# nkargas/Gen2-UHF-RFID-Reader

Measured on AMD Instinct MI355X. Metric: I/Q Msamples/s through matched_filter->gate->tag_decoder (+ EPC decodes/s), 40 kHz FM0, higher is better.
Workload: dtype f32; 1 GPU; configs[1]: batch of 1024 noise-replicas per GPU of the 71-round file_source_test stand-in trace, FM0 40 kHz BLF @ 2 Msps (1076066 raw I/Q samples each, sigma=0.002), generated and resident in HBM; streams_per_gpu=1024, hbm_bytes_traces=8815132672, parallelism=traces sharded per GPU, no collective

## Files before the change

gen2-uhf-rfid-reader_amd/csrc/rfid_capi.hip:

```cpp
#include <hip/hip_runtime.h>

#include <cmath>
#include <ctime>
#include <pthread.h>
#include <cstdio>
#include <cstdlib>
#include <cstring>
#include <deque>
#include <initializer_list>
#include <map>
#include <memory>
#include <new>
#include <vector>

#include "rfid_host_math.h"
#include "rfid_kernels.hpp"
#include "rfid_inventory.hpp"
#include "rfid_tracks.hpp"
#include "rfid_quality.hpp"
#include "rfid_mi355x.h"
#include "rfid_gen2_host.h"
#define LS2_LAUNCH(kernel, gx, gy, block, args) \
  hipLaunchKernelGGL(rfidk::kernel, dim3((unsigned)(gx), (unsigned)(gy)), dim3((unsigned)(block)), 0, ls2_stream, args)
static thread_local hipStream_t ls2_stream = nullptr;
static thread_local unsigned ls2_front_lds = 0;
#define LS2_LAUNCH_FRONT(kernel, gx, gy, block, args) \
  hipLaunchKernelGGL(rfidk::kernel, dim3((unsigned)(gx), (unsigned)(gy)), dim3((unsigned)(block)), ls2_front_lds, ls2_stream, args)
static double g_la_t[20] = {0};
static long g_la_n[20] = {0};
static bool g_la_on = false;
static inline void la_count(int k, double dt) { if (g_la_on) { g_la_t[k] += dt; g_la_n[k]++; } }
static inline double la_now() { struct timespec ts; clock_gettime(CLOCK_MONOTONIC, &ts); return 1e3 * (double)ts.tv_sec + 1e-6 * (double)ts.tv_nsec; }
struct LaTimer { int k; double t0; explicit LaTimer(int kk) : k(kk), t0(g_la_on ? la_now() : 0.0) {} ~LaTimer() { if (g_la_on) la_count(k, la_now() - t0); } };
#include "rfid_ls2_enqueue.hpp"

using namespace rfidk;

namespace {

struct DevBuf {
  void *p = nullptr;
  size_t cap = 0;
};

}

struct RfidKnobs {
  int long_stream = 1;
  int overlap = 1;
  int ls_calibrate = 1;
  int ls_debug = 0;
  int la_profile = 0;
  int front_unfused = 0;
  int front_chunks = 1;
  int fsm_lanes_min = -1;
  int dc_rounds = -1;
  int la_upload_kernel = 1;
  int front_lds_kb = -1;
  int inventory_slots = 0;
};

struct rfid_ctx {
  rfid_params prm;
  RfidKnobs knobs;
  int device = 0;
  hipStream_t stream = nullptr;
  char err[512];
  float t_cand[N_TCAND];

  rfid_reader_state rs;

  void *d_small = nullptr;
  GateState *d_gate1 = nullptr;
  int *d_io = nullptr;
  DevBuf s_in, s_out;
  DevBuf synth_tab;
  DevBuf ls2_ws;
  DevBuf ls2_ws_alt;
  bool ls2_mark_failed = false;
  bool y_touched = false;
  Ls2Ctl *ls2_host = nullptr;
  Ls2Ctl *d_ls2_ctl = nullptr;
  int ls2_P = 0;
  int ls2_rounds[3] = {0, 0, 0};
  bool ls2_generous = false;
  int ls_mode = 1;
// ... 184 lines not shown
  float front_ms = 0.0f;
};

namespace {

void sio_free(rfid_ctx *c);
int sio_process(rfid_ctx *c, int b, int64_t n_new, bool flush);
int sio_submit(rfid_ctx *c, int b, int64_t n_new, bool flush);
int sio_collect(rfid_ctx *c);
void la_free(rfid_ctx *c);
int la_mf_work(rfid_ctx *c, const rfid_cf32 *in, int n_in, rfid_cf32 *out, int out_cap, int *n_produced);
int la_gate_work(rfid_ctx *c, const rfid_cf32 *in, int n_in, rfid_cf32 *out, int out_cap, int *n_consumed, int *n_written);
int la_gate_swallow(rfid_ctx *c, const rfid_cf32 *in, int n_in, rfid_cf32 *out, int out_cap, int *n_consumed, int *n_written);
bool la_decoder_result(rfid_ctx *c, const rfid_cf32 *in, int wlen, int type, rfid_decode_result *r);

int fail(rfid_ctx *c, int code, const char *what, hipError_t e = hipSuccess) {
  if (c) {
    if (e != hipSuccess)
      snprintf(c->err, sizeof(c->err), "%s: %s", what, hipGetErrorString(e));
    else
      snprintf(c->err, sizeof(c->err), "%s", what);
  }
  return code;
}

struct KnobEntry { const char *name, *env; int RfidKnobs::*field; int lo, hi; };
const KnobEntry g_knob_table[] = {
  {"long_stream", "RFID_LONG_STREAM", &RfidKnobs::long_stream, 0, 2},
  {"overlap", "RFID_OVERLAP", &RfidKnobs::overlap, 0, 2},
  {"ls_calibrate", "RFID_LS_CALIBRATE", &RfidKnobs::ls_calibrate, 0, 1},
  {"ls_debug", "RFID_LS_DEBUG", &RfidKnobs::ls_debug, 0, 1},
  {"la_profile", "RFID_LA_PROFILE", &RfidKnobs::la_profile, 0, 1},
  {"front_unfused", "RFID_FRONT_UNFUSED", &RfidKnobs::front_unfused, 0, 1},
  {"front_chunks", "RFID_FRONT_CHUNKS", &RfidKnobs::front_chunks, 1, rfid_ctx::MAX_CHUNKS},
  {"fsm_lanes_min", "RFID_LS2_FSM_LANES_MIN", &RfidKnobs::fsm_lanes_min, -1, 1 << 30},
  {"dc_rounds", "RFID_LS2_DC_ROUNDS", &RfidKnobs::dc_rounds, -1, 64},
  {"la_upload_kernel", "RFID_LA_UPLOAD_KERNEL", &RfidKnobs::la_upload_kernel, 0, 1},
  {"front_lds_kb", "RFID_LS_FRONT_LDS_KB", &RfidKnobs::front_lds_kb, -1, 64},
  {"inventory_slots", "RFID_INVENTORY_SLOTS", &RfidKnobs::inventory_slots, 0, 1024},
};
int clamp_int(long v, int lo, int hi) { return (int)(v < lo ? lo : (v > hi ? hi : v)); }
void knobs_from_env(RfidKnobs &k) {
  for (const KnobEntry &e : g_knob_table) {
    const char *v = getenv(e.env);
    if (!v || !*v) continue;
    char *end = nullptr;
    const long x = strtol(v, &end, 10);
    if (end == v) continue;
    k.*(e.field) = clamp_int(x, e.lo, e.hi);
  }
}

#define HIPCHK(c, call)                                                     \
  do {                                                                      \
    hipError_t e__ = (call);                                                \
    if (e__ != hipSuccess) return fail((c), RFID_ERR_HIP, #call, e__);      \
  } while (0)

#define HIPCHK_T(c, call)                                                   \
  do {                                                                      \
    hipError_t e__ = (call);                                                \
    if (e__ != hipSuccess) { (c)->y_touched = true; return fail((c), RFID_ERR_HIP, #call, e__); } \
  } while (0)

int grow(rfid_ctx *c, DevBuf &b, size_t bytes) {
  if (bytes <= b.cap) return RFID_OK;
// ... 1286 lines not shown
  }
  c->d_ls2_ctl = nullptr;
  c->y_touched = true;
  if (nch < 2 && raw_stride >= 2 && !c->knobs.front_unfused) {
    HIPCHK(c, hipSetDevice(c->device));
    c->d_lens = (const int64_t *)d_lens;
    c->last_n_raw = n_raw;
    c->n_chunks_last = 0;
    const bool overlap = c->alt_have && !want_scores;
    if (overlap) {
      std::swap(c->d_y, c->alt.d_y); std::swap(c->d_wtab, c->alt.d_wtab); std::swap(c->d_flat, c->alt.d_flat);
      std::swap(c->d_wcount, c->alt.d_wcount); std::swap(c->d_flat_count, c->alt.d_flat_count);
      std::swap(c->d_res, c->alt.d_res); std::swap(c->d_stats, c->alt.d_stats);
      c->set_idx ^= 1;
      if (c->tail_recorded[c->set_idx]) {
        HIPCHK(c, hipStreamWaitEvent(c->stream, c->ev_tail_done[c->set_idx], 0));
        c->tail_recorded[c->set_idx] = false;
      }
    } else {
      int rj = join_tails(c);
      if (rj) return rj;
    }
    HIPCHK(c, hipEventRecord(c->ev[0], c->stream));
    HIPCHK(c, hipEventRecord(c->ev[1], c->stream));
    HIPCHK(c, hipMemsetAsync(c->d_gstate, 0, sizeof(GateState) * (size_t)c->B, c->stream));
    HIPCHK(c, hipMemsetAsync(c->d_flat_count, 0, 2 * sizeof(int), c->stream));
    GateArgs g = {};
    g.y = c->d_y; g.y_w = c->d_y; g.y_stride = c->y_stride; g.n_dec = n_out; g.lens = c->d_lens;
    g.pos0 = 0; g.chunk_len = n_out;
    g.state = c->d_gstate; g.n_streams = c->B; g.wtab = c->d_wtab; g.wmax = c->wmax; g.wcount = c->d_wcount;
    g.flat = c->d_flat; g.flat_count = c->d_flat_count; g.flat_cap = c->flat_cap; g.mode = 0;
    g.raw = (const float2 *)d_raw; g.raw_stride = raw_stride; g.n_raw = n_raw;
    g.raw_vec_ok = ((raw_stride & 1) == 0 && (((uintptr_t)d_raw) & 15) == 0) ? 1 : 0;
    hipLaunchKernelGGL(front_end_fused_kernel, dim3((unsigned)((c->B + GATE_STREAMS_PER_WG - 1) / GATE_STREAMS_PER_WG)),
                       dim3(GATE_THREADS), 0, c->stream, g);
    HIPCHK(c, hipGetLastError());
    HIPCHK(c, hipEventRecord(c->ev[2], c->stream));
    c->ev_valid[0] = c->ev_valid[1] = c->ev_valid[2] = true;
    c->fused_last = 1;
    if (overlap) {
      HIPCHK(c, hipEventRecord(c->ev_fe_done, c->stream));
      HIPCHK(c, hipStreamWaitEvent(c->stream2, c->ev_fe_done, 0));
      c->tail_stream = c->stream2;
      c->ev_valid[2] = false;
      int rc = rfid_batch_decode(c, 0);
      if (!rc) rc = rfid_batch_stats(c);
      c->tail_stream = nullptr;
      if (rc) return rc;
      HIPCHK(c, hipEventRecord(c->ev_tail_done[c->set_idx], c->stream2));
      c->tail_recorded[c->set_idx] = true;
      return RFID_OK;
    }
    int rc = rfid_batch_decode(c, want_scores);
    if (rc) return rc;
    return rfid_batch_stats(c);
  }
  c->fused_last = 0;
  if (tiles < 4 * (int64_t)nch || nch < 2) {
    int rc = rfid_batch_mf(c, d_raw, raw_stride, n_raw, d_lens);
    if (rc) return rc;
    if ((rc = rfid_batch_gate(c))) return rc;
    if ((rc = rfid_batch_decode(c, want_scores))) return rc;
    return rfid_batch_stats(c);
  }
  HIPCHK(c, hipSetDevice(c->device));
  { int rj = join_tails(c); if (rj) return rj; }
// ... 660 lines not shown
```

gen2-uhf-rfid-reader_amd/csrc/rfid_kernels.hpp:

```cpp
#pragma once
#include <rfid_device_env.h>
#include "rfid_mi355x.h"

namespace rfidk {

constexpr int DECIM = 5;
constexpr int NTAPS = 25;
constexpr int WIN_LEN = 100;
constexpr int DC_LEN = 48;
constexpr int T1_SAMPLES = 96;
constexpr int PW_HALF = 2;
constexpr int GATE_N_SAT = 128;
static_assert(GATE_N_SAT > T1_SAMPLES && GATE_N_SAT > PW_HALF, "the saturated count must pass every comparison");
constexpr int NUM_PULSES_CMD = 5;
constexpr int RN16_WIN = 250;
constexpr int EPC_WIN = 1370;
constexpr int N_SYNC = 15;
constexpr int N_TCAND = 20;
constexpr float HALF_BIT = 5.0f;
constexpr float WIN_LEN_F = 100.0f;
constexpr float DC_LEN_F = 48.0f;
constexpr float THRESH_FRACTION = 0.75f;

constexpr int MF_TILE = 512;
// ... 165 lines not shown
  int win_index;
  int dc_index;
  int win_seq;
  float win[WIN_LEN];
  float dcr_re[DC_LEN];
  float dcr_im[DC_LEN];
};

struct GateArgs {
  const float2 *y;
  int64_t y_stride;
  int64_t n_dec;
  int64_t pos0;
  int64_t chunk_len;
  const int64_t *lens;
  GateState *state;
  int n_streams;
  rfid_window *wtab;
  int wmax;
  int *wcount;
  rfid_window *flat;
  int *flat_count;
  int flat_cap;
  int mode;
  float2 *gated;
  int gated_cap;
  int *io;
  const float2 *raw;
  int64_t raw_stride;
  int64_t n_raw;
  int raw_vec_ok;
  float2 *y_w;
  const int *skip_if;
};

RFID_DEVICE bool div_const_ok(float x) {
  const uint32_t u = wv::f2u(x);
  return ((u & 0x7fffffffu) - 0x0d800000u) < (0x7f800000u - 0x0d800000u) || u == 0u;
}
template <int C>
RFID_DEVICE float div_const_fast(float x) {
  constexpr float c = (float)C, rc = 1.0f / (float)C;
  const float q1 = x * rc;
  return wv::fma_f(wv::fma_f(-q1, c, x), rc, q1);
}
RFID_DEVICE uint64_t div_const_bad(float x) {
  const uint32_t u = wv::f2u(x);
  return wv::ballot(((u & 0x7fffffffu) - 0x0d800000u) >= (0x7f800000u - 0x0d800000u)) & wv::ballot(u != 0u);
}
template <int C>
RFID_DEVICE float div_const(float x) {
  if (__builtin_expect(div_const_bad(x) == 0, 1)) return div_const_fast<C>(x);
  return wv::fdiv(x, (float)C);
}

RFID_DEVICE float chain_add(float carry, float x, int lane) {
  const float x0 = (lane == 0) ? (carry + x) : x;
  float p = x0;
#pragma unroll
  for (int s = 1; s < 64; ++s) p = wv::shr1(p) + x0;
  return p;
}

RFID_DEVICE uint64_t prefix_xor64(uint64_t x) {
  x ^= x << 1; x ^= x << 2; x ^= x << 4; x ^= x << 8; x ^= x << 16; x ^= x << 32;
  return x;
// ... 364 lines not shown
  return used_spec;
}
RFID_DEVICE void chain_add2_ends(float &cr, float &ci, const float *re, const float *im, int lane) {
  const float4 *src = reinterpret_cast<const float4 *>((lane & 1) ? im : re);
  float4 v[16];
#pragma unroll
  for (int j = 0; j < 16; ++j) v[j] = src[j];
  float sum = (lane & 1) ? ci : cr;
#pragma unroll
  for (int j = 0; j < 16; ++j) {
    sum = sum + v[j].x;
    sum = sum + v[j].y;
    sum = sum + v[j].z;
    sum = sum + v[j].w;
  }
  cr = wv::readlane(sum, 0);
  ci = wv::readlane(sum, 1);
}
template <bool SCAN, class Spec>
RFID_DEVICE void gate_dc_step(GateBackRegs &g, uint64_t closedmask, uint64_t openmask, int nvalid, float2 yv, int lane,
                              float2 *lds_dc, float2 *lds_tmp, Spec spec, float &dcr, float &dci, bool spec_ok = true) {
  float tre, tim;
  gate_dc_incr(g, closedmask, openmask, nvalid, yv, lane, lds_dc, lds_tmp, spec, tre, tim, spec_ok);
  if (SCAN) {
    dcr = chain_add_auto(g.dcr_c, tre, lane);
    dci = chain_add_auto(g.dci_c, tim, lane);
  } else {
    chain_add2(g.dcr_c, tre, g.dci_c, tim, lane, dcr, dci);
  }
  g.dcr_c = wv::readlane(dcr, 63);
  g.dci_c = wv::readlane(dci, 63);
}

RFID_DEVICE void gate_back(const GateArgs &a, GateBackRegs &g, const GateSlot *slot, int pos, int n_total, int row, int lane,
                           float2 *lds_dc, float2 *lds_tmp, bool &stop) {
  int word, w1 = 0;
  uint64_t closedmask, openmask;
  const int spec_bad_v = wv::lds_peek(&slot->spec_bad);
  wv::lds_load_rec(&slot->b_word, word, closedmask);
  const int flags = word & 7, nvalid = (word >> 8) & 0xff, open = (word >> 16) & 0x1ff;
  if (a.mode != 0) wv::lds_load_rec(reinterpret_cast<const int *>(&slot->b_openmask), w1, openmask);
  else openmask = (flags & 4) ? 1ull : 0ull;
  const bool spec_ok = wv::uniform(spec_bad_v) == 0;
  float dcr, dci;
  const bool lanes_wanted = (open & 0xff) != 0xff || a.mode == 1;
  if ((flags & 1) && !lanes_wanted) {
    float tre = 0.0f, tim = 0.0f;
    const bool spec = gate_dc_incr(g, closedmask, openmask, nvalid, slot->yv[lane], lane, lds_dc, lds_tmp,
                                   [&](float &, float &) {}, tre, tim, spec_ok);
    const float *re = slot->tre, *im = slot->tim;
    if (!spec) {
      float *t = reinterpret_cast<float *>(lds_tmp);
      t[lane] = tre; t[64 + lane] = tim;
      wv::wave_sync();
      re = t; im = t + 64;
    }
    chain_add2_ends(g.dcr_c, g.dci_c, re, im, lane);
    dcr = g.dcr_c; dci = g.dci_c;
  } else if (flags & 1) {
    gate_dc_step<false>(g, closedmask, openmask, nvalid, slot->yv[lane], lane, lds_dc, lds_tmp,
                 [&](float &tre, float &tim) { tre = slot->tre[lane]; tim = slot->tim[lane]; }, dcr, dci, spec_ok);
  } else {
    g.run_closed = 0;
    dcr = g.dcr_c; dci = g.dci_c;
  }
  const int open_lane = open & 0xff;
  if (__builtin_expect(open_lane != 0xff, 0))
    gate_record_window(a, g, open_lane, (open >> 8) & 1, pos, n_total, row, lane, dcr, dci);
  if (__builtin_expect(a.mode == 1, 0)) {
    if (openmask != 0) {
      const uint64_t lt = (lane == 0) ? 0ull : (~0ull >> (64 - lane));
      const float2 yv = slot->yv[lane];
      const bool isopen = ((openmask >> lane) & 1ull) != 0;
      const int orank = wv::popc64(openmask & lt);
      if (isopen && g.written + orank < a.gated_cap)
        a.gated[g.written + orank] = make_float2(yv.x - dcr, yv.y - dci);
      g.written += wv::popc64(openmask);
    }
  }
  stop = (flags & 2) != 0;
}

constexpr int GATE_RAW = 64 * DECIM + (NTAPS - DECIM);
constexpr int GATE_RAW4 = GATE_RAW / 2;
constexpr int GATE_RAW_LD = (GATE_RAW4 + 63) / 64;
constexpr int GATE_RAW_DEPTH = 6;
constexpr int GATE_STREAMS_PER_WG = 4;
constexpr int GATE_ROLES = 4;
constexpr int GATE_THREADS = 64 * GATE_ROLES * GATE_STREAMS_PER_WG;
constexpr int GATE_WAVES_PER_SIMD = 4;
constexpr int GATE_SLOTS = 16;
constexpr int GATE_PREFETCH = 4;

struct GateShared {
  GateSlot slots[GATE_SLOTS];
  float win[WIN_LEN + 4];
  float2 dc[DC_LEN];
  alignas(16) float2 tmp[64];
  float4 rawtile[64 * GATE_RAW_LD];
  int fir_seq;
  int prod_seq;
  int fsm_seq;
  int back_seq;
  int stop;
  int fsm_done;
  int prod_done;
};

struct GateRawRegs {
  float4 v[GATE_RAW_LD];
};

struct GateTrue { static constexpr bool value = true; };
// ... 17 lines not shown
  hrel = (hrel < -(1 << 30)) ? -(1 << 30) : hrel;
  const int hi = (int)hrel;
#pragma unroll
  for (int j = 0; j < GATE_RAW_LD; ++j) {
    int q = lane + 64 * j;
    q = (q < GATE_RAW4) ? q : (GATE_RAW4 - 1);
    int ri = 2 * q;
    ri = (ri < lo) ? lo : ri;
    ri = (ri > hi) ? hi : ri;
    if (vec) {
      r.v[j] = *reinterpret_cast<const float4 *>(p + ri);
    } else {
      const float2 lo2 = p[ri], hi2 = p[ri + 1];
      r.v[j] = make_float4(lo2.x, lo2.y, hi2.x, hi2.y);
    }
  }
}

RFID_DEVICE float2 gate_fir_step(const GateRawRegs &r, float4 *tile4, int lane, bool first) {
  wv::wave_sync();
#pragma unroll
  for (int j = 0; j < GATE_RAW_LD; ++j) {
    const int q = lane + 64 * j;
    float4 v = r.v[j];
    if (j == 0 && first && q < (NTAPS - 1) / 2) v = make_float4(0.0f, 0.0f, 0.0f, 0.0f);
    tile4[q] = v;
  }
  wv::wave_sync();
  const float2 *tile = reinterpret_cast<const float2 *>(tile4);
  static_assert(NTAPS == 25, "lds_sum25_in_order");
  return wv::lds_sum25_in_order(&tile[DECIM * lane]);
}

template <bool FUSED>
RFID_DEVICE void gate_scan_body(const GateArgs &a) {
  RFID_SHARED GateShared sh_all[GATE_STREAMS_PER_WG];
  const int lane = wv::lane_id();
  const int wave = wv::uniform((int)(threadIdx.x >> 6));
  const int role = wave / GATE_STREAMS_PER_WG;
  const int sl = wave % GATE_STREAMS_PER_WG;
  const int s = (int)blockIdx.x * GATE_STREAMS_PER_WG + sl;
  GateShared &sh = sh_all[sl];
  if (lane == 0 && role == 0) {
    sh.fir_seq = 0; sh.prod_seq = 0; sh.fsm_seq = 0; sh.back_seq = 0; sh.stop = 0; sh.fsm_done = 0; sh.prod_done = 0;
  }
  wv::block_sync();
  if (s >= a.n_streams) return;
  if (a.skip_if && wv::uniform(*a.skip_if) != 0) return;
  const int strm = s, row = s;
  const int64_t pos0 = a.pos0, chunk_len = a.chunk_len;
  GateState *st = a.state + row;
  const float2 *ys = a.y + (int64_t)strm * a.y_stride + pos0;
  int64_t n64 = a.n_dec;
  if (a.lens) {
    int64_t r = a.lens[strm];
    if (r < 0) r = 0;
    n64 = r / DECIM;
    if (n64 > a.n_dec) n64 = a.n_dec;
  }
  const int n_total = wv::uniform((int)n64);
  int64_t nl = n64 - pos0;
  if (nl > chunk_len) nl = chunk_len;
  if (nl < 0) nl = 0;
  const int n = wv::uniform((int)nl);
  const int nsteps = (n + 63) >> 6;
  const int win_index0 = wv::uniform(st->win_index);

  if (role == 1) {
    bool stopped = false;
    float2 prev_yv = make_float2(0.0f, 0.0f);
    if (FUSED) {
      const float2 *xs = a.raw + (int64_t)strm * a.raw_stride;
      const bool vec = a.raw_vec_ok != 0;
      const int64_t hi_idx = vec ? ((a.raw_stride - 2) & ~(int64_t)1) : (a.raw_stride - 2);
      float2 *yw = a.y_w + (int64_t)strm * a.y_stride + pos0;
      const int64_t rbase = pos0 * DECIM - (NTAPS - 1);
      const int nfull = n >> 6;
      const int ngroups = nfull / GATE_RAW_DEPTH;
      const bool at_start = pos0 == 0;
      int back_seen = 0;
      if (ngroups > 0) {
        GateRawRegs buf[GATE_RAW_DEPTH];
#pragma unroll
        for (int u = 0; u < GATE_RAW_DEPTH; ++u) {
          gate_load_raw(buf[u], xs, hi_idx, rbase + (int64_t)u * 64 * DECIM, lane, vec);
          wv::compiler_fence();
        }
        int g_fast = 0;
        if (vec) {
          const int64_t j_max = (hi_idx - 2 * (GATE_RAW4 - 1) - rbase) / (64 * DECIM);
          int64_t gf = (j_max + 1) / GATE_RAW_DEPTH - 1;
          gf = (gf < 0) ? 0 : gf;
          g_fast = (gf > ngroups) ? ngroups : (int)gf;
        }
        auto group = [&](int grp, auto interior) {
#pragma unroll
          for (int u = 0; u < GATE_RAW_DEPTH; ++u) {
            const int k = grp * GATE_RAW_DEPTH + u;
            while (k - back_seen >= GATE_SLOTS) { back_seen = wv::lds_load(&sh.back_seq); if (k - back_seen >= GATE_SLOTS) wv::backoff(); }
            const float2 yv = gate_fir_step(buf[u], sh.rawtile, lane, u == 0 && grp == 0 && at_start);
            gate_load_raw<decltype(interior)::value>(buf[u], xs, hi_idx, rbase + (int64_t)(k + GATE_RAW_DEPTH) * 64 * DECIM, lane, vec);
            yw[64 * k + lane] = yv;
            sh.slots[k % GATE_SLOTS].yv[lane] = yv;
            gate_spec_dc(sh.slots[k % GATE_SLOTS], yv, prev_yv, lane);
            wv::lds_store(&sh.fir_seq, k + 1, lane);
          }
        };
        int grp = 0;
        for (; grp < g_fast; ++grp) group(grp, GateTrue());
        for (; grp < ngroups; ++grp) group(grp, GateFalse());
      }
      for (int k = ngroups * GATE_RAW_DEPTH; k < nsteps; ++k) {
        while (k - back_seen >= GATE_SLOTS) { back_seen = wv::lds_load(&sh.back_seq); if (k - back_seen >= GATE_SLOTS) wv::backoff(); }
        GateRawRegs r;
        gate_load_raw(r, xs, hi_idx, rbase + (int64_t)k * 64 * DECIM, lane, vec);
        float2 yv = gate_fir_step(r, sh.rawtile, lane, k == 0 && at_start);
        if (64 * k + lane < n) yw[64 * k + lane] = yv;
        else yv = make_float2(0.0f, 0.0f);
        sh.slots[k % GATE_SLOTS].yv[lane] = yv;
        gate_spec_dc(sh.slots[k % GATE_SLOTS], yv, prev_yv, lane);
        wv::lds_store(&sh.fir_seq, k + 1, lane);
      }
      wv::global_release();
    } else {
      float2 cur[GATE_PREFETCH], nxt[GATE_PREFETCH];
#pragma unroll
      for (int u = 0; u < GATE_PREFETCH; ++u) {
        const int i = 64 * u + lane;
        cur[u] = (i < n) ? ys[i] : make_float2(0.0f, 0.0f);
      }
      for (int base = 0; base < nsteps && !stopped; base += GATE_PREFETCH) {
#pragma unroll
        for (int u = 0; u < GATE_PREFETCH; ++u) {
          const int i = 64 * (base + GATE_PREFETCH + u) + lane;
          nxt[u] = (i < n) ? ys[i] : make_float2(0.0f, 0.0f);
        }
#pragma unroll
        for (int u = 0; u < GATE_PREFETCH; ++u) {
          const int k = base + u;
          if (k < nsteps && !stopped) {
            while (!stopped && k - wv::lds_load(&sh.back_seq) >= GATE_SLOTS) {
              stopped = wv::lds_load(&sh.stop) != 0;
              wv::backoff();
            }
            if (!stopped) {
              sh.slots[k % GATE_SLOTS].yv[lane] = cur[u];
              gate_spec_dc(sh.slots[k % GATE_SLOTS], cur[u], prev_yv, lane);
              wv::lds_store(&sh.fir_seq, k + 1, lane);
            }
          }
        }
#pragma unroll
        for (int u = 0; u < GATE_PREFETCH; ++u) cur[u] = nxt[u];
      }
    }
    wv::lds_store(&sh.prod_done, 1, lane);
  } else if (role == 3) {
    for (int j = lane; j < WIN_LEN; j += 64) sh.win[j] = st->win[j];
    int win_index = win_index0;
    wv::wave_sync();
    bool stopped = false;
    int fir_seen = 0;
    for (int k = 0; k < nsteps && !stopped; ++k) {
      while (!stopped && fir_seen <= k) {
        fir_seen = wv::lds_load(&sh.fir_seq);
        if (fir_seen <= k) {
          stopped = wv::lds_load(&sh.stop) != 0;
          wv::backoff();
        }
      }
      if (!stopped) {
        GateSlot &slot = sh.slots[k % GATE_SLOTS];
        gate_produce(slot, slot.yv[lane], 64 * k, n, lane, sh.win, win_index);
        wv::lds_store(&sh.prod_seq, k + 1, lane);
      }
    }
  } else if (role == 2) {
    float2 *lds_dc = sh.dc, *lds_tmp = sh.tmp;
    if (lane < DC_LEN) lds_dc[lane] = make_float2(st->dcr_re[lane], st->dcr_im[lane]);
    GateBackRegs g;
    g.dcr_c = wv::uniform(st->dc_re); g.dci_c = wv::uniform(st->dc_im);
    g.dc_index = wv::uniform(st->dc_index);
    g.run_closed = 0; g.ring_stale = 0;
    g.prev_yv = make_float2(0.0f, 0.0f);
    g.win_seq = wv::uniform(st->win_seq);
    g.n_complete = 0; g.written = 0;
    g.pos0 = (int)pos0; g.strm = strm;
    wv::wave_sync();
    bool stop = false;
    int fsm_seen = 0;
    for (int k = 0; k < nsteps && !stop; ++k) {
      bool have = true;
      while (fsm_seen <= k) {
        fsm_seen = wv::lds_load(&sh.fsm_seq);
        if (fsm_seen > k) break;
        if (wv::lds_load(&sh.fsm_done) != 0) {
          fsm_seen = wv::lds_load(&sh.fsm_seq);
          if (fsm_seen <= k) { have = false; break; }
        } else {
          wv::backoff();
        }
      }
      if (!have) break;
      gate_back(a, g, &sh.slots[k % GATE_SLOTS], 64 * k, n_total, row, lane, lds_dc, lds_tmp, stop);
      wv::lds_store(&sh.back_seq, k + 1, lane);
    }
    if (g.ring_stale) {
      if (lane >= 64 - DC_LEN) {
        int di = g.dc_index + (lane - (64 - DC_LEN));
        if (di >= DC_LEN) di -= DC_LEN;
        lds_dc[di] = g.prev_yv;
      }
      wv::wave_sync();
    }
    if (lane < DC_LEN) { st->dcr_re[lane] = lds_dc[lane].x; st->dcr_im[lane] = lds_dc[lane].y; }
    if (lane == 0) {
      st->dc_re = g.dcr_c; st->dc_im = g.dci_c; st->win_seq = g.win_seq; st->dc_index = g.dc_index;
      if (a.mode != 0) a.io[1] = g.written;
    }
    if (a.mode == 0) {
      const int before = (pos0 > 0) ? wv::uniform(a.wcount[row]) : 0;
      int tot = before + g.n_complete;
      tot = (tot < a.wmax) ? tot : a.wmax;
      if (lane == 0) a.wcount[row] = tot;
      gate_flat_lists(a, row, before, tot - before, lane);
    }
  } else {
    wv::set_priority_high();
    GateRegs g;
    g.avg_c = wv::uniform(st->avg_ampl);
    g.f_n = wv::uniform(st->n_samples); g.f_state = wv::uniform(st->signal_state);
    g.f_pulses = wv::uniform(st->num_pulses); g.f_open = wv::uniform(st->gate_open);
    g.f_ung = wv::uniform(st->n_to_ungate); g.f_type = wv::uniform(st->wtype);
    if (g.f_ung == 0) g.f_ung = g.f_type ? EPC_WIN : RN16_WIN;
    g.consumed = n; g.stop = false;
    GateNext nx;
    nx.step = -1; nx.sq = 0; nx.amp = nx.d = 0.0f;
    for (int k = 0; k < nsteps && !g.stop; ++k) {
      gate_consume(a, g, &sh.slots[k % GATE_SLOTS], &sh.slots[(k + 1) % GATE_SLOTS], nx, &sh.prod_seq, k, 64 * k, n, lane);
      wv::lds_store(&sh.fsm_seq, k + 1, lane);
      wv::lds_prefetch_wait<2>(nx.sq, nx.amp, nx.d);
    }
    wv::lds_store(&sh.fsm_done, 1, lane);
    if (g.stop) wv::lds_store(&sh.stop, 1, lane);

    while (wv::lds_load(&sh.prod_done) == 0) wv::backoff();
    {
      const int c = g.consumed;
      const int first = (c > WIN_LEN) ? (c - WIN_LEN) : 0;
      for (int i = first + lane; i < c; i += 64) {
        const float2 v = FUSED ? wv::load_coherent(&ys[i]) : ys[i];
        st->win[(win_index0 + i) % WIN_LEN] = wv::hypot_f(v.x, v.y);
      }
    }
    if (lane == 0) {
      st->avg_ampl = g.avg_c;
      st->n_samples = g.f_n; st->signal_state = g.f_state; st->num_pulses = g.f_pulses;
      st->gate_open = g.f_open; st->n_to_ungate = g.f_ung; st->wtype = g.f_type;
      st->win_index = (win_index0 + g.consumed) % WIN_LEN;
      if (a.mode != 0) a.io[0] = g.consumed;
    }
  }
}

RFID_KERNEL_OCC(GATE_THREADS, GATE_WAVES_PER_SIMD) void gate_scan_kernel(GateArgs a) { gate_scan_body<false>(a); }
RFID_KERNEL_OCC(GATE_THREADS, GATE_WAVES_PER_SIMD) void front_end_fused_kernel(GateArgs a) { gate_scan_body<true>(a); }

constexpr int LS_QUIET = EPC_WIN + T1_SAMPLES + 1 + WIN_LEN + DC_LEN;
static_assert(GATE_N_SAT < WIN_LEN + DC_LEN - 1, "n_samples must have saturated at every cut (147 samples after a window at least)");

struct LsCutArgs {
  const float2 *y;
  int64_t y_stride;
  const int64_t *lens;
  int64_t n_dec;
  int chunk;
  int limit;
  int max_b;
  int quiet;
  int *cut;
};

RFID_DEVICE void ls_cut_body(const LsCutArgs &a, const int s, const int j) {
  const int lane = wv::lane_id();
  int64_t n64 = a.n_dec;
  if (a.lens) { int64_t r = a.lens[s]; if (r < 0) r = 0; n64 = r / DECIM; if (n64 > a.n_dec) n64 = a.n_dec; }
  const int n = (int)n64;
  const int P = j * a.chunk;
  int *out = a.cut + (int64_t)s * a.max_b + j;
  if (P >= n) { if (lane == 0) *out = -1; return; }
  const float2 *ys = a.y + (int64_t)s * a.y_stride;
  int lo = P - a.quiet - 64;
  if (lo < 0) lo = 0;
  float ref = 0.0f;
  for (int base = lo; base < P; base += 64) {
    const int i = base + lane;
    float m2 = 0.0f;
    if (i < P) { const float2 v = ys[i]; m2 = v.x * v.x + v.y * v.y; }
    ref = (m2 > ref) ? m2 : ref;
// ... 998 lines not shown
```

Measured before the change: 412,400 Msamples/s.

## Process gate pipeline in pairs of 64-sample steps in the fused front end

Adds a paired-step variant of the fused front-end kernel in which the FIR, amplitude, FSM and DC-back waves each handle two 64-sample steps per handshake. The FSM also gets a two-step chained-add scan. This halves the LDS sequence polling and synchronisation per sample and lets the back stage skip pairs with no closed windows. It is on by default in mode 0, with the old single-step path kept behind a knob. The price is more code and register pressure, plus possible rounding and tie-handling edge cases in the paired scan.

```diff
diff --git a/gen2-uhf-rfid-reader_amd/csrc/rfid_capi.hip b/gen2-uhf-rfid-reader_amd/csrc/rfid_capi.hip
--- a/gen2-uhf-rfid-reader_amd/csrc/rfid_capi.hip
+++ b/gen2-uhf-rfid-reader_amd/csrc/rfid_capi.hip
@@ -52,6 +52,7 @@
   int ls_debug = 0;
   int la_profile = 0;
   int front_unfused = 0;
+  int front_single_step = 0;
   int front_chunks = 1;
   int fsm_lanes_min = -1;
   int dc_rounds = -1;
@@ -302,6 +303,7 @@
   {"ls_debug", "RFID_LS_DEBUG", &RfidKnobs::ls_debug, 0, 1},
   {"la_profile", "RFID_LA_PROFILE", &RfidKnobs::la_profile, 0, 1},
   {"front_unfused", "RFID_FRONT_UNFUSED", &RfidKnobs::front_unfused, 0, 1},
+  {"front_single_step", "RFID_FRONT_SINGLE_STEP", &RfidKnobs::front_single_step, 0, 1},
   {"front_chunks", "RFID_FRONT_CHUNKS", &RfidKnobs::front_chunks, 1, rfid_ctx::MAX_CHUNKS},
   {"fsm_lanes_min", "RFID_LS2_FSM_LANES_MIN", &RfidKnobs::fsm_lanes_min, -1, 1 << 30},
   {"dc_rounds", "RFID_LS2_DC_ROUNDS", &RfidKnobs::dc_rounds, -1, 64},
@@ -1654,6 +1656,7 @@
     g.flat = c->d_flat; g.flat_count = c->d_flat_count; g.flat_cap = c->flat_cap; g.mode = 0;
     g.raw = (const float2 *)d_raw; g.raw_stride = raw_stride; g.n_raw = n_raw;
     g.raw_vec_ok = ((raw_stride & 1) == 0 && (((uintptr_t)d_raw) & 15) == 0) ? 1 : 0;
+    g.single_step = c->knobs.front_single_step;
     hipLaunchKernelGGL(front_end_fused_kernel, dim3((unsigned)((c->B + GATE_STREAMS_PER_WG - 1) / GATE_STREAMS_PER_WG)),
                        dim3(GATE_THREADS), 0, c->stream, g);
     HIPCHK(c, hipGetLastError());
diff --git a/gen2-uhf-rfid-reader_amd/csrc/rfid_kernels.hpp b/gen2-uhf-rfid-reader_amd/csrc/rfid_kernels.hpp
--- a/gen2-uhf-rfid-reader_amd/csrc/rfid_kernels.hpp
+++ b/gen2-uhf-rfid-reader_amd/csrc/rfid_kernels.hpp
@@ -221,6 +221,7 @@
   int raw_vec_ok;
   float2 *y_w;
   const int *skip_if;
+  int single_step;
 };
 
 RFID_DEVICE bool div_const_ok(float x) {
@@ -651,15 +652,10 @@
   g.dci_c = wv::readlane(dci, 63);
 }
 
-RFID_DEVICE void gate_back(const GateArgs &a, GateBackRegs &g, const GateSlot *slot, int pos, int n_total, int row, int lane,
-                           float2 *lds_dc, float2 *lds_tmp, bool &stop) {
-  int word, w1 = 0;
-  uint64_t closedmask, openmask;
-  const int spec_bad_v = wv::lds_peek(&slot->spec_bad);
-  wv::lds_load_rec(&slot->b_word, word, closedmask);
+RFID_DEVICE void gate_back_desc(const GateArgs &a, GateBackRegs &g, const GateSlot *slot, int word, uint64_t closedmask,
+                                uint64_t openmask, int spec_bad_v, int pos, int n_total, int row, int lane,
+                                float2 *lds_dc, float2 *lds_tmp, bool &stop) {
   const int flags = word & 7, nvalid = (word >> 8) & 0xff, open = (word >> 16) & 0x1ff;
-  if (a.mode != 0) wv::lds_load_rec(reinterpret_cast<const int *>(&slot->b_openmask), w1, openmask);
-  else openmask = (flags & 4) ? 1ull : 0ull;
   const bool spec_ok = wv::uniform(spec_bad_v) == 0;
   float dcr, dci;
   const bool lanes_wanted = (open & 0xff) != 0xff || a.mode == 1;
@@ -698,6 +694,16 @@
     }
   }
   stop = (flags & 2) != 0;
+}
+RFID_DEVICE void gate_back(const GateArgs &a, GateBackRegs &g, const GateSlot *slot, int pos, int n_total, int row, int lane,
+                           float2 *lds_dc, float2 *lds_tmp, bool &stop) {
+  int word, w1 = 0;
+  uint64_t closedmask, openmask;
+  const int spec_bad_v = wv::lds_peek(&slot->spec_bad);
+  wv::lds_load_rec(&slot->b_word, word, closedmask);
+  if (a.mode != 0) wv::lds_load_rec(reinterpret_cast<const int *>(&slot->b_openmask), w1, openmask);
+  else openmask = (word & 4) ? 1ull : 0ull;
+  gate_back_desc(a, g, slot, word, closedmask, openmask, spec_bad_v, pos, n_total, row, lane, lds_dc, lds_tmp, stop);
 }
 
 constexpr int GATE_RAW = 64 * DECIM + (NTAPS - DECIM);
@@ -781,9 +787,107 @@
   return wv::lds_sum25_in_order(&tile[DECIM * lane]);
 }
 
+RFID_DEVICE GateShared *gate_shared() {
+  RFID_SHARED GateShared sh_all[GATE_STREAMS_PER_WG];
+  return sh_all;
+}
+
+struct GateExtent { int n_total, n, nsteps; };
+RFID_DEVICE GateExtent gate_extent(const GateArgs &a, int strm) {
+  int64_t n64 = a.n_dec;
+  if (a.lens) {
+    int64_t r = a.lens[strm];
+    if (r < 0) r = 0;
+    n64 = r / DECIM;
+    if (n64 > a.n_dec) n64 = a.n_dec;
+  }
+  GateExtent e;
+  e.n_total = wv::uniform((int)n64);
+  int64_t nl = n64 - a.pos0;
+  if (nl > a.chunk_len) nl = a.chunk_len;
+  if (nl < 0) nl = 0;
+  e.n = wv::uniform((int)nl);
+  e.nsteps = (e.n + 63) >> 6;
+  return e;
+}
+RFID_DEVICE void gate_filter_tail(GateShared &sh, const float2 *xs, int64_t hi_idx, int64_t rbase, bool vec, float2 *yw, int k0,
+                                  int nsteps, int n, bool at_start, int &back_seen, float2 &prev_yv, int lane) {
+  for (int k = k0; k < nsteps; ++k) {
+    while (k - back_seen >= GATE_SLOTS) { back_seen = wv::lds_load(&sh.back_seq); if (k - back_seen >= GATE_SLOTS) wv::backoff(); }
+    GateRawRegs r;
+    gate_load_raw(r, xs, hi_idx, rbase + (int64_t)k * 64 * DECIM, lane, vec);
+    float2 yv = gate_fir_step(r, sh.rawtile, lane, k == 0 && at_start);
+    if (64 * k + lane < n) yw[64 * k + lane] = yv;
+    else yv = make_float2(0.0f, 0.0f);
+    sh.slots[k % GATE_SLOTS].yv[lane] = yv;
+    gate_spec_dc(sh.slots[k % GATE_SLOTS], yv, prev_yv, lane);
+    wv::lds_store(&sh.fir_seq, k + 1, lane);
+  }
+}
+RFID_DEVICE void gate_back_begin(GateBackRegs &g, const GateState *st, float2 *lds_dc, int64_t pos0, int strm, int lane) {
+  if (lane < DC_LEN) lds_dc[lane] = make_float2(st->dcr_re[lane], st->dcr_im[lane]);
+  g.dcr_c = wv::uniform(st->dc_re); g.dci_c = wv::uniform(st->dc_im);
+  g.dc_index = wv::uniform(st->dc_index);
+  g.run_closed = 0; g.ring_stale = 0;
+  g.prev_yv = make_float2(0.0f, 0.0f);
+  g.win_seq = wv::uniform(st->win_seq);
+  g.n_complete = 0; g.written = 0;
+  g.pos0 = (int)pos0; g.strm = strm;
+  wv::wave_sync();
+}
+RFID_DEVICE void gate_back_end(const GateArgs &a, GateBackRegs &g, GateState *st, float2 *lds_dc, int row, int64_t pos0, int lane) {
+  if (g.ring_stale) {
+    if (lane >= 64 - DC_LEN) {
+      int di = g.dc_index + (lane - (64 - DC_LEN));
+      if (di >= DC_LEN) di -= DC_LEN;
+      lds_dc[di] = g.prev_yv;
+    }
+    wv::wave_sync();
+  }
+  if (lane < DC_LEN) { st->dcr_re[lane] = lds_dc[lane].x; st->dcr_im[lane] = lds_dc[lane].y; }
+  if (lane == 0) {
+    st->dc_re = g.dcr_c; st->dc_im = g.dci_c; st->win_seq = g.win_seq; st->dc_index = g.dc_index;
+    if (a.mode != 0) a.io[1] = g.written;
+  }
+  if (a.mode == 0) {
+    const int before = (pos0 > 0) ? wv::uniform(a.wcount[row]) : 0;
+    int tot = before + g.n_complete;
+    tot = (tot < a.wmax) ? tot : a.wmax;
+    if (lane == 0) a.wcount[row] = tot;
+    gate_flat_lists(a, row, before, tot - before, lane);
+  }
+}
+RFID_DEVICE void gate_fsm_begin(GateRegs &g, const GateState *st, int n) {
+  g.avg_c = wv::uniform(st->avg_ampl);
+  g.f_n = wv::uniform(st->n_samples); g.f_state = wv::uniform(st->signal_state);
+  g.f_pulses = wv::uniform(st->num_pulses); g.f_open = wv::uniform(st->gate_open);
+  g.f_ung = wv::uniform(st->n_to_ungate); g.f_type = wv::uniform(st->wtype);
+  if (g.f_ung == 0) g.f_ung = g.f_type ? EPC_WIN : RN16_WIN;
+  g.consumed = n; g.stop = false;
+}
+template <bool FUSED>
+RFID_DEVICE void gate_fsm_end(const GateArgs &a, const GateRegs &g, GateState *st, GateShared &sh, const float2 *ys, int win_index0, int lane) {
+  while (wv::lds_load(&sh.prod_done) == 0) wv::backoff();
+  {
+    const int c = g.consumed;
+    const int first = (c > WIN_LEN) ? (c - WIN_LEN) : 0;
+    for (int i = first + lane; i < c; i += 64) {
+      const float2 v = FUSED ? wv::load_coherent(&ys[i]) : ys[i];
+      st->win[(win_index0 + i) % WIN_LEN] = wv::hypot_f(v.x, v.y);
+    }
+  }
+  if (lane == 0) {
+    st->avg_ampl = g.avg_c;
+    st->n_samples = g.f_n; st->signal_state = g.f_state; st->num_pulses = g.f_pulses;
+    st->gate_open = g.f_open; st->n_to_ungate = g.f_ung; st->wtype = g.f_type;
+    st->win_index = (win_index0 + g.consumed) % WIN_LEN;
+    if (a.mode != 0) a.io[0] = g.consumed;
+  }
+}
+
 template <bool FUSED>
 RFID_DEVICE void gate_scan_body(const GateArgs &a) {
-  RFID_SHARED GateShared sh_all[GATE_STREAMS_PER_WG];
+  GateShared *sh_all = gate_shared();
   const int lane = wv::lane_id();
   const int wave = wv::uniform((int)(threadIdx.x >> 6));
   const int role = wave / GATE_STREAMS_PER_WG;
@@ -797,22 +901,11 @@
   if (s >= a.n_streams) return;
   if (a.skip_if && wv::uniform(*a.skip_if) != 0) return;
   const int strm = s, row = s;
-  const int64_t pos0 = a.pos0, chunk_len = a.chunk_len;
+  const int64_t pos0 = a.pos0;
   GateState *st = a.state + row;
   const float2 *ys = a.y + (int64_t)strm * a.y_stride + pos0;
-  int64_t n64 = a.n_dec;
-  if (a.lens) {
-    int64_t r = a.lens[strm];
-    if (r < 0) r = 0;
-    n64 = r / DECIM;
-    if (n64 > a.n_dec) n64 = a.n_dec;
-  }
-  const int n_total = wv::uniform((int)n64);
-  int64_t nl = n64 - pos0;
-  if (nl > chunk_len) nl = chunk_len;
-  if (nl < 0) nl = 0;
-  const int n = wv::uniform((int)nl);
-  const int nsteps = (n + 63) >> 6;
+  const GateExtent ex = gate_extent(a, strm);
+  const int n_total = ex.n_total, n = ex.n, nsteps = ex.nsteps;
   const int win_index0 = wv::uniform(st->win_index);
 
   if (role == 1) {
@@ -859,17 +952,7 @@
         for (; grp < g_fast; ++grp) group(grp, GateTrue());
         for (; grp < ngroups; ++grp) group(grp, GateFalse());
       }
-      for (int k = ngroups * GATE_RAW_DEPTH; k < nsteps; ++k) {
-        while (k - back_seen >= GATE_SLOTS) { back_seen = wv::lds_load(&sh.back_seq); if (k - back_seen >= GATE_SLOTS) wv::backoff(); }
-        GateRawRegs r;
-        gate_load_raw(r, xs, hi_idx, rbase + (int64_t)k * 64 * DECIM, lane, vec);
-        float2 yv = gate_fir_step(r, sh.rawtile, lane, k == 0 && at_start);
-        if (64 * k + lane < n) yw[64 * k + lane] = yv;
-        else yv = make_float2(0.0f, 0.0f);
-        sh.slots[k % GATE_SLOTS].yv[lane] = yv;
-        gate_spec_dc(sh.slots[k % GATE_SLOTS], yv, prev_yv, lane);
-        wv::lds_store(&sh.fir_seq, k + 1, lane);
-      }
+      gate_filter_tail(sh, xs, hi_idx, rbase, vec, yw, ngroups * GATE_RAW_DEPTH, nsteps, n, at_start, back_seen, prev_yv, lane);
       wv::global_release();
     } else {
       float2 cur[GATE_PREFETCH], nxt[GATE_PREFETCH];
@@ -926,16 +1009,8 @@
     }
   } else if (role == 2) {
     float2 *lds_dc = sh.dc, *lds_tmp = sh.tmp;
-    if (lane < DC_LEN) lds_dc[lane] = make_float2(st->dcr_re[lane], st->dcr_im[lane]);
     GateBackRegs g;
-    g.dcr_c = wv::uniform(st->dc_re); g.dci_c = wv::uniform(st->dc_im);
-    g.dc_index = wv::uniform(st->dc_index);
-    g.run_closed = 0; g.ring_stale = 0;
-    g.prev_yv = make_float2(0.0f, 0.0f);
-    g.win_seq = wv::uniform(st->win_seq);
-    g.n_complete = 0; g.written = 0;
-    g.pos0 = (int)pos0; g.strm = strm;
-    wv::wave_sync();
+    gate_back_begin(g, st, lds_dc, pos0, strm, lane);
     bool stop = false;
     int fsm_seen = 0;
     for (int k = 0; k < nsteps && !stop; ++k) {
@@ -954,35 +1029,11 @@
       gate_back(a, g, &sh.slots[k % GATE_SLOTS], 64 * k, n_total, row, lane, lds_dc, lds_tmp, stop);
       wv::lds_store(&sh.back_seq, k + 1, lane);
     }
-    if (g.ring_stale) {
-      if (lane >= 64 - DC_LEN) {
-        int di = g.dc_index + (lane - (64 - DC_LEN));
-        if (di >= DC_LEN) di -= DC_LEN;
-        lds_dc[di] = g.prev_yv;
-      }
-      wv::wave_sync();
-    }
-    if (lane < DC_LEN) { st->dcr_re[lane] = lds_dc[lane].x; st->dcr_im[lane] = lds_dc[lane].y; }
-    if (lane == 0) {
-      st->dc_re = g.dcr_c; st->dc_im = g.dci_c; st->win_seq = g.win_seq; st->dc_index = g.dc_index;
-      if (a.mode != 0) a.io[1] = g.written;
-    }
-    if (a.mode == 0) {
-      const int before = (pos0 > 0) ? wv::uniform(a.wcount[row]) : 0;
-      int tot = before + g.n_complete;
-      tot = (tot < a.wmax) ? tot : a.wmax;
-      if (lane == 0) a.wcount[row] = tot;
-      gate_flat_lists(a, row, before, tot - before, lane);
-    }
+    gate_back_end(a, g, st, lds_dc, row, pos0, lane);
   } else {
     wv::set_priority_high();
     GateRegs g;
-    g.avg_c = wv::uniform(st->avg_ampl);
-    g.f_n = wv::uniform(st->n_samples); g.f_state = wv::uniform(st->signal_state);
-    g.f_pulses = wv::uniform(st->num_pulses); g.f_open = wv::uniform(st->gate_open);
-    g.f_ung = wv::uniform(st->n_to_ungate); g.f_type = wv::uniform(st->wtype);
-    if (g.f_ung == 0) g.f_ung = g.f_type ? EPC_WIN : RN16_WIN;
-    g.consumed = n; g.stop = false;
+    gate_fsm_begin(g, st, n);
     GateNext nx;
     nx.step = -1; nx.sq = 0; nx.amp = nx.d = 0.0f;
     for (int k = 0; k < nsteps && !g.stop; ++k) {
@@ -993,27 +1044,299 @@
     wv::lds_store(&sh.fsm_done, 1, lane);
     if (g.stop) wv::lds_store(&sh.stop, 1, lane);
 
-    while (wv::lds_load(&sh.prod_done) == 0) wv::backoff();
+    gate_fsm_end<FUSED>(a, g, st, sh, ys, win_index0, lane);
+  }
+}
+
+struct ScanHalf {
+  float frac;
+  bool tie;
+  int R;
+  uint64_t badmask_t, tiemask;
+};
+RFID_DEVICE void scan_half_round(float x, float scale, uint32_t sign, ScanHalf &h) {
+  const float t = sign ? -(x * scale) : (x * scale);
+  const float r = wv::rint_f(t);
+  h.frac = t - r;
+  const bool bad_t = !(__builtin_fabsf(t) < 4194304.0f);
+  const bool half = __builtin_fabsf(h.frac) == 0.5f;
+  h.tie = !bad_t && half;
+  h.R = wv::f2i(bad_t ? 0.0f : r);
+  h.badmask_t = wv::ballot(bad_t);
+  h.tiemask = wv::ballot(half) & ~h.badmask_t;
+}
+RFID_DEVICE uint32_t scan_half_ties(ScanHalf &h, uint32_t cin, int lane) {
+  const int I = h.R - ((h.frac < 0.0f) ? 1 : 0);
+  const uint64_t rodd = wv::ballot((h.R & 1) != 0) & ~h.tiemask;
+  const uint64_t iodd = wv::ballot((I & 1) != 0) & h.tiemask;
+  const uint64_t Q = prefix_xor64(rodd);
+  const uint64_t gen = h.tiemask & Q, X = gen | ~h.tiemask;
+  const uint64_t sum = X + gen + (uint64_t)(cin & 1u);
+  const uint64_t W = X ^ gen ^ sum;
+  const uint64_t par = (Q << 1) ^ W;
+  const uint64_t up = (par ^ iodd) & h.tiemask;
+  h.R = h.tie ? (I + (int)((up >> lane) & 1ull)) : h.R;
+  return (h.tiemask >> 63) ? 0u : (uint32_t)(((par ^ rodd) >> 63) & 1ull);
+}
+RFID_DEVICE bool chain_add_scan_pair(float carry, float x0, float x1, int lane, float &out0, float &out1) {
+  const uint32_t cb = wv::f2u(carry);
+  const uint32_t e_b = (cb >> 23) & 0xffu;
+  const uint32_t sign = cb & 0x80000000u;
+  const float scale = wv::u2f(((277u - e_b) & 0xffu) << 23);
+  ScanHalf h0, h1;
+  scan_half_round(x0, scale, sign, h0);
+  scan_half_round(x1, scale, sign, h1);
+  if ((h0.tiemask | h1.tiemask) != 0ull) {
+    uint32_t par = cb & 1u;
+    if (h0.tiemask != 0ull) par = scan_half_ties(h0, par, lane);
+    else par ^= (uint32_t)wv::popc64(wv::ballot((h0.R & 1) != 0)) & 1u;
+    if (h1.tiemask != 0ull) scan_half_ties(h1, par, lane);
+  }
+  const int s0 = wv::scan_add(h0.R), s1 = wv::scan_add(h1.R);
+  const uint32_t base = cb & 0x7fffffffu;
+  const uint32_t mag0 = base + (uint32_t)s0;
+  const uint32_t mag1 = base + (uint32_t)wv::readlane(s0, 63) + (uint32_t)s1;
+  const uint64_t badmask_s = wv::ballot((((mag0 ^ cb) | (mag1 ^ cb)) & 0x7f800000u) != 0u) |
+                             wv::ballot((mag0 & 0x007fffffu) == 0u) | wv::ballot((mag1 & 0x007fffffu) == 0u);
+  const bool bad_c = e_b < 23u || e_b > 254u;
+  out0 = wv::u2f(mag0 | sign);
+  out1 = wv::u2f(mag1 | sign);
+  return (h0.badmask_t | h1.badmask_t | badmask_s) == 0ull && !bad_c;
+}
+
+RFID_DEVICE void gate_produce_pair(GateSlot &s0, GateSlot &s1, float2 yv0, float2 yv1, int lane, float *lds_win, int &win_index) {
+  const float amp0 = wv::hypot_f(yv0.x, yv0.y);
+  const float amp1 = wv::hypot_f(yv1.x, yv1.y);
+  int wi0 = win_index + lane;
+  if (wi0 >= WIN_LEN) wi0 -= WIN_LEN;
+  int wi1 = wi0 + 64;
+  if (wi1 >= WIN_LEN) wi1 -= WIN_LEN;
+  const float old0 = lds_win[wi0];
+  wv::wave_sync();
+  lds_win[wi0] = amp0;
+  wv::wave_sync();
+  const float old1 = lds_win[wi1];
+  wv::wave_sync();
+  lds_win[wi1] = amp1;
+  wv::wave_sync();
+  static_assert(WIN_LEN == 100, "128 mod WIN_LEN");
+  win_index += 128 - WIN_LEN;
+  if (win_index >= WIN_LEN) win_index -= WIN_LEN;
+  const float nd0 = amp0 - old0, nd1 = amp1 - old1;
+  float d0, d1;
+  if (__builtin_expect((div_const_bad(nd0) | div_const_bad(nd1)) == 0ull, 1)) {
+    d0 = div_const_fast<WIN_LEN>(nd0); d1 = div_const_fast<WIN_LEN>(nd1);
+  } else {
+    d0 = wv::fdiv(nd0, (float)WIN_LEN); d1 = wv::fdiv(nd1, (float)WIN_LEN);
+  }
+  s0.amp[lane] = amp0; s0.d[lane] = d0;
+  s1.amp[lane] = amp1; s1.d[lane] = d1;
+}
+
+struct GateNextPair {
+  int step;
+  int sq;
+  float amp0, d0, amp1, d1;
+};
+RFID_DEVICE void gate_fetch_pair(GateNextPair &nx, const int *seq, const GateSlot *s0, const GateSlot *s1, int k, int lane) {
+  wv::compiler_fence();
+  nx.sq = wv::lds_peek(seq);
+  wv::compiler_fence();
+  nx.amp0 = s0->amp[lane]; nx.d0 = s0->d[lane];
+  nx.amp1 = s1->amp[lane]; nx.d1 = s1->d[lane];
+  wv::compiler_fence();
+  nx.step = k;
+}
+RFID_DEVICE void gate_consume_pair(GateRegs &g, GateSlot *s0, GateSlot *s1, const GateSlot *n0, const GateSlot *n1,
+                                   GateNextPair &nx, const int *seq, int k, int lane) {
+  if (!(nx.step == k && wv::uniform(nx.sq) > k + 1)) {
+    while (wv::lds_load(seq) <= k + 1) wv::backoff();
+    gate_fetch_pair(nx, seq, s0, s1, k, lane);
+  }
+  const float f_amp0 = nx.amp0, f_d0 = nx.d0, f_amp1 = nx.amp1, f_d1 = nx.d1;
+  float avg0, avg1;
+  if (__builtin_expect(!chain_add_scan_pair(g.avg_c, f_d0, f_d1, lane, avg0, avg1), 0)) {
+    avg0 = chain_add_auto(g.avg_c, f_d0, lane);
+    avg1 = chain_add_auto(wv::readlane(avg0, 63), f_d1, lane);
+  }
+  g.avg_c = wv::readlane(avg1, 63);
+  const float th0 = avg0 * THRESH_FRACTION, th1 = avg1 * THRESH_FRACTION;
+  const uint64_t below0 = wv::ballot(f_amp0 < th0), below1 = wv::ballot(f_amp1 < th1);
+  gate_fetch_pair(nx, seq, n0, n1, k + 2, lane);
+  uint64_t closed0, open0, closed1, open1;
+  int ol0 = 0xff, ot0 = 0, ol1 = 0xff, ot1 = 0;
+  const bool plain_open = g.f_open && (g.f_ung - g.f_n > 128);
+  const bool plain_closed = !g.f_open && (g.f_state == 1) && ((below0 | below1) == 0) &&
+                            !((g.f_pulses > NUM_PULSES_CMD) && (T1_SAMPLES - g.f_n < 128));
+  if (__builtin_expect(plain_open || plain_closed, 1)) {
+    g.f_n += 128;
+    closed0 = closed1 = plain_closed ? ~0ull : 0ull;
+    open0 = open1 = plain_closed ? 0ull : ~0ull;
+    if (!g.f_open && g.f_n > GATE_N_SAT) g.f_n = GATE_N_SAT;
+  } else {
+    const uint64_t above0 = wv::ballot(f_amp0 > th0), above1 = wv::ballot(f_amp1 > th1);
+    int nv = 64;
+    gate_fsm_step(0, g, below0, above0, 64 * k, nv, closed0, open0, ol0, ot0);
+    nv = 64;
+    gate_fsm_step(0, g, below1, above1, 64 * k + 64, nv, closed1, open1, ol1, ot1);
+  }
+  wv::lds_store_rec(&s0->b_word, ((closed0 != 0) ? 1 : 0) | ((open0 != 0) ? 4 : 0) | (64 << 8) | (ol0 << 16) | (ot0 << 24), closed0, lane);
+  wv::lds_store_rec(&s1->b_word, ((closed1 != 0) ? 1 : 0) | ((open1 != 0) ? 4 : 0) | (64 << 8) | (ol1 << 16) | (ot1 << 24), closed1, lane);
+}
+
+RFID_DEVICE void gate_back_pair(const GateArgs &a, GateBackRegs &g, const GateSlot *s0, const GateSlot *s1, int pos, int n_total,
+                                int row, int lane, float2 *lds_dc, float2 *lds_tmp) {
+  int word0, word1;
+  uint64_t closed0, closed1;
+  const int sb0 = wv::lds_peek(&s0->spec_bad), sb1 = wv::lds_peek(&s1->spec_bad);
+  wv::lds_load_rec(&s0->b_word, word0, closed0);
+  wv::lds_load_rec(&s1->b_word, word1, closed1);
+  if (((word0 | word1) & 1) == 0) {
+    g.run_closed = 0;
+    return;
+  }
+  bool stop;
+  gate_back_desc(a, g, s0, word0, closed0, (word0 & 4) ? 1ull : 0ull, sb0, pos, n_total, row, lane, lds_dc, lds_tmp, stop);
+  gate_back_desc(a, g, s1, word1, closed1, (word1 & 4) ? 1ull : 0ull, sb1, pos + 64, n_total, row, lane, lds_dc, lds_tmp, stop);
+}
+
+RFID_DEVICE void gate_pairs_body(const GateArgs &a) {
+  GateShared *sh_all = gate_shared();
+  const int lane = wv::lane_id();
+  const int wave = wv::uniform((int)(threadIdx.x >> 6));
+  const int role = wave / GATE_STREAMS_PER_WG;
+  const int sl = wave % GATE_STREAMS_PER_WG;
+  const int s = (int)blockIdx.x * GATE_STREAMS_PER_WG + sl;
+  GateShared &sh = sh_all[sl];
+  if (lane == 0 && role == 0) {
+    sh.fir_seq = 0; sh.prod_seq = 0; sh.fsm_seq = 0; sh.back_seq = 0; sh.stop = 0; sh.fsm_done = 0; sh.prod_done = 0;
+  }
+  wv::block_sync();
+  if (s >= a.n_streams) return;
+  if (a.skip_if && wv::uniform(*a.skip_if) != 0) return;
+  const int strm = s, row = s;
+  const int64_t pos0 = a.pos0;
+  GateState *st = a.state + row;
+  const float2 *ys = a.y + (int64_t)strm * a.y_stride + pos0;
+  const GateExtent ex = gate_extent(a, strm);
+  const int n_total = ex.n_total, n = ex.n, nsteps = ex.nsteps;
+  const int nfull = n >> 6;
+  const int npaired = nfull & ~1;
+  const int win_index0 = wv::uniform(st->win_index);
+
+  if (role == 1) {
+    float2 prev_yv = make_float2(0.0f, 0.0f);
+    const float2 *xs = a.raw + (int64_t)strm * a.raw_stride;
+    const bool vec = a.raw_vec_ok != 0;
+    const int64_t hi_idx = vec ? ((a.raw_stride - 2) & ~(int64_t)1) : (a.raw_stride - 2);
+    float2 *yw = a.y_w + (int64_t)strm * a.y_stride + pos0;
+    const int64_t rbase = pos0 * DECIM - (NTAPS - 1);
+    static_assert(GATE_RAW_DEPTH % 2 == 0 && GATE_SLOTS % 2 == 0, "a group is whole pairs, a pair does not straddle the ring's wrap");
+    const int ngroups = nfull / GATE_RAW_DEPTH;
+    const bool at_start = pos0 == 0;
+    int back_seen = 0;
+    if (ngroups > 0) {
+      GateRawRegs buf[GATE_RAW_DEPTH];
+#pragma unroll
+      for (int u = 0; u < GATE_RAW_DEPTH; ++u) {
+        gate_load_raw(buf[u], xs, hi_idx, rbase + (int64_t)u * 64 * DECIM, lane, vec);
+        wv::compiler_fence();
+      }
+      int g_fast = 0;
+      if (vec) {
+        const int64_t j_max = (hi_idx - 2 * (GATE_RAW4 - 1) - rbase) / (64 * DECIM);
+        int64_t gf = (j_max + 1) / GATE_RAW_DEPTH - 1;
+        gf = (gf < 0) ? 0 : gf;
+        g_fast = (gf > ngroups) ? ngroups : (int)gf;
+      }
+      auto group = [&](int grp, auto interior) {
+#pragma unroll
+        for (int u = 0; u < GATE_RAW_DEPTH; ++u) {
+          const int k = grp * GATE_RAW_DEPTH + u;
+          if ((u & 1) == 0)
+            while (k + 1 - back_seen >= GATE_SLOTS) { back_seen = wv::lds_load(&sh.back_seq); if (k + 1 - back_seen >= GATE_SLOTS) wv::backoff(); }
+          const float2 yv = gate_fir_step(buf[u], sh.rawtile, lane, u == 0 && grp == 0 && at_start);
+          gate_load_raw<decltype(interior)::value>(buf[u], xs, hi_idx, rbase + (int64_t)(k + GATE_RAW_DEPTH) * 64 * DECIM, lane, vec);
+          yw[64 * k + lane] = yv;
+          sh.slots[k % GATE_SLOTS].yv[lane] = yv;
+          gate_spec_dc(sh.slots[k % GATE_SLOTS], yv, prev_yv, lane);
+          if ((u & 1) == 1) wv::lds_store(&sh.fir_seq, k + 1, lane);
+        }
+      };
+      int grp = 0;
+      for (; grp < g_fast; ++grp) group(grp, GateTrue());
+      for (; grp < ngroups; ++grp) group(grp, GateFalse());
+    }
+    gate_filter_tail(sh, xs, hi_idx, rbase, vec, yw, ngroups * GATE_RAW_DEPTH, nsteps, n, at_start, back_seen, prev_yv, lane);
+    wv::global_release();
+    wv::lds_store(&sh.prod_done, 1, lane);
+  } else if (role == 3) {
+    for (int j = lane; j < WIN_LEN; j += 64) sh.win[j] = st->win[j];
+    int win_index = win_index0;
+    wv::wave_sync();
+    int fir_seen = 0;
+    int k = 0;
+    for (; k < npaired; k += 2) {
+      while (fir_seen <= k + 1) { fir_seen = wv::lds_load(&sh.fir_seq); if (fir_seen <= k + 1) wv::backoff(); }
+      GateSlot &s0 = sh.slots[k % GATE_SLOTS], &s1 = sh.slots[k % GATE_SLOTS + 1];
+      gate_produce_pair(s0, s1, s0.yv[lane], s1.yv[lane], lane, sh.win, win_index);
+      wv::lds_store(&sh.prod_seq, k + 2, lane);
+    }
+    for (; k < nsteps; ++k) {
+      while (fir_seen <= k) { fir_seen = wv::lds_load(&sh.fir_seq); if (fir_seen <= k) wv::backoff(); }
+      GateSlot &slot = sh.slots[k % GATE_SLOTS];
+      gate_produce(slot, slot.yv[lane], 64 * k, n, lane, sh.win, win_index);
+      wv::lds_store(&sh.prod_seq, k + 1, lane);
+    }
+  } else if (role == 2) {
+    float2 *lds_dc = sh.dc, *lds_tmp = sh.tmp;
+    GateBackRegs g;
+    gate_back_begin(g, st, lds_dc, pos0, strm, lane);
+    int fsm_seen = 0;
+    int k = 0;
+    for (; k < npaired; k += 2) {
+      while (fsm_seen <= k + 1) { fsm_seen = wv::lds_load(&sh.fsm_seq); if (fsm_seen <= k + 1) wv::backoff(); }
+      gate_back_pair(a, g, &sh.slots[k % GATE_SLOTS], &sh.slots[k % GATE_SLOTS + 1], 64 * k, n_total, row, lane, lds_dc, lds_tmp);
+      wv::lds_store(&sh.back_seq, k + 2, lane);
+    }
+    for (; k < nsteps; ++k) {
+      while (fsm_seen <= k) { fsm_seen = wv::lds_load(&sh.fsm_seq); if (fsm_seen <= k) wv::backoff(); }
+      bool stop;
+      gate_back(a, g, &sh.slots[k % GATE_SLOTS], 64 * k, n_total, row, lane, lds_dc, lds_tmp, stop);
+      wv::lds_store(&sh.back_seq, k + 1, lane);
+    }
+    gate_back_end(a, g, st, lds_dc, row, pos0, lane);
+  } else {
+    wv::set_priority_high();
+    GateRegs g;
+    gate_fsm_begin(g, st, n);
+    int k = 0;
     {
-      const int c = g.consumed;
-      const int first = (c > WIN_LEN) ? (c - WIN_LEN) : 0;
-      for (int i = first + lane; i < c; i += 64) {
-        const float2 v = FUSED ? wv::load_coherent(&ys[i]) : ys[i];
-        st->win[(win_index0 + i) % WIN_LEN] = wv::hypot_f(v.x, v.y);
-      }
-    }
-    if (lane == 0) {
-      st->avg_ampl = g.avg_c;
-      st->n_samples = g.f_n; st->signal_state = g.f_state; st->num_pulses = g.f_pulses;
-      st->gate_open = g.f_open; st->n_to_ungate = g.f_ung; st->wtype = g.f_type;
-      st->win_index = (win_index0 + g.consumed) % WIN_LEN;
-      if (a.mode != 0) a.io[0] = g.consumed;
-    }
+      GateNextPair nx;
+      nx.step = -1; nx.sq = 0; nx.amp0 = nx.d0 = nx.amp1 = nx.d1 = 0.0f;
+      for (; k < npaired; k += 2) {
+        GateSlot *s0 = &sh.slots[k % GATE_SLOTS], *n0 = &sh.slots[(k + 2) % GATE_SLOTS];
+        gate_consume_pair(g, s0, s0 + 1, n0, n0 + 1, nx, &sh.prod_seq, k, lane);
+        wv::lds_store(&sh.fsm_seq, k + 2, lane);
+      }
+    }
+    GateNext nx;
+    nx.step = -1; nx.sq = 0; nx.amp = nx.d = 0.0f;
+    for (; k < nsteps; ++k) {
+      gate_consume(a, g, &sh.slots[k % GATE_SLOTS], &sh.slots[(k + 1) % GATE_SLOTS], nx, &sh.prod_seq, k, 64 * k, n, lane);
+      wv::lds_store(&sh.fsm_seq, k + 1, lane);
+      wv::lds_prefetch_wait<2>(nx.sq, nx.amp, nx.d);
+    }
+    wv::lds_store(&sh.fsm_done, 1, lane);
+    gate_fsm_end<true>(a, g, st, sh, ys, win_index0, lane);
   }
 }
 
 RFID_KERNEL_OCC(GATE_THREADS, GATE_WAVES_PER_SIMD) void gate_scan_kernel(GateArgs a) { gate_scan_body<false>(a); }
-RFID_KERNEL_OCC(GATE_THREADS, GATE_WAVES_PER_SIMD) void front_end_fused_kernel(GateArgs a) { gate_scan_body<true>(a); }
+RFID_KERNEL_OCC(GATE_THREADS, GATE_WAVES_PER_SIMD) void front_end_fused_kernel(GateArgs a) {
+  if (a.single_step == 0 && a.mode == 0) gate_pairs_body(a);
+  else gate_scan_body<true>(a);
+}
 
 constexpr int LS_QUIET = EPC_WIN + T1_SAMPLES + 1 + WIN_LEN + DC_LEN;
 static_assert(GATE_N_SAT < WIN_LEN + DC_LEN - 1, "n_samples must have saturated at every cut (147 samples after a window at least)");
```

Measured after the change: 439,400 Msamples/s (median of 6 runs). 1.07x the previous value.
